# shenyunhang/JTSM

Measured on AMD Instinct MI355X. Metric: images/sec training, R50-FPN JTSM panoptic, 2x1024x1024, 1/2/4/8 GPU, higher is better.
Workload: dtype bf16x3; 1 GPU; BASELINE configs[2]: JTSM panoptic R50-FPN, 2 x 3x1024x1024 per GPU, 2000 proposals + 1024 superpixels per image; MIL + 4 OICR + 2 mask heads + sem-seg; fwd + bwd + gradient exchange + SGD; 100% of proposals jittered copies of 40 rectangles per image; global_batch=2, parallelism=dp1, foreground_rois_last_step=281

## Files before the change

include/jtsm_hip.h:

```cpp
#ifndef JTSM_HIP_H_
#define JTSM_HIP_H_

#include <stddef.h>
#include <stdint.h>

#ifdef __cplusplus
extern "C" {
#endif

#define JTSM_OK 0
#define JTSM_EINVAL (-1)
#define JTSM_ELAUNCH (-2)
#define JTSM_ENODEV (-3)

#define JTSM_NCHW 0
#define JTSM_NHWC 1

const char* jtsm_last_error(void);
const char* jtsm_version(void);
int jtsm_device_count(void);

void* jtsm_event_create(void);
int jtsm_event_record(void* event, void* stream);
int jtsm_event_elapsed_ms(void* start, void* stop, float* ms);
void jtsm_event_destroy(void* event);
void jtsm_conv_set_mid_event(void* event);
void jtsm_conv_set_splitk_fused(int mode);

int jtsm_roi_align_forward_f32(const float* input, const float* rois, float* output, int B,
                               int C, int H, int W, int M, float spatial_scale, int pooled_h,
                               int pooled_w, int sampling_ratio, int aligned, int layout,
                               void* stream);
int jtsm_roi_align_backward_f32(const float* grad, const float* rois, float* grad_input, int B,
                                int C, int H, int W, int M, float spatial_scale, int pooled_h,
                                int pooled_w, int sampling_ratio, int aligned, int layout,
                                void* stream);
int jtsm_roi_align_forward_f64(const double* input, const double* rois, double* output, int B,
                               int C, int H, int W, int M, double spatial_scale, int pooled_h,
                               int pooled_w, int sampling_ratio, int aligned, int layout,
                               void* stream);
int jtsm_roi_align_backward_f64(const double* grad, const double* rois, double* grad_input,
                                int B, int C, int H, int W, int M, double spatial_scale,
                                int pooled_h, int pooled_w, int sampling_ratio, int aligned,
                                int layout, void* stream);

int jtsm_roi_align_rotated_forward_f32(const float* input, const float* rois, float* output,
                                       int B, int C, int H, int W, int M, float spatial_scale,
                                       int pooled_h, int pooled_w, int sampling_ratio,
                                       int layout, void* stream);
int jtsm_roi_align_rotated_backward_f32(const float* grad, const float* rois, float* grad_input,
                                        int B, int C, int H, int W, int M, float spatial_scale,
                                        int pooled_h, int pooled_w, int sampling_ratio,
                                        int layout, void* stream);
int jtsm_roi_align_rotated_forward_f64(const double* input, const double* rois, double* output,
                                       int B, int C, int H, int W, int M, double spatial_scale,
                                       int pooled_h, int pooled_w, int sampling_ratio,
                                       int layout, void* stream);
int jtsm_roi_align_rotated_backward_f64(const double* grad, const double* rois,
                                        double* grad_input, int B, int C, int H, int W, int M,
                                        double spatial_scale, int pooled_h, int pooled_w,
                                        int sampling_ratio, int layout, void* stream);

int jtsm_roi_sample_table_f32(const float* rois, int rotated, int M, int H, int W,
                              float spatial_scale, int pooled_h, int pooled_w,
                              int sampling_ratio, int aligned, int* grid, int* pos, float* w,
                              int cap, void* stream);

size_t jtsm_moi_pool_workspace_bytes(int B, int H, int W, int M, int L);
int jtsm_moi_pool_forward_f32(const float* input, const float* rois, const int32_t* oh_labels,
                              const int32_t* superpixels, float* output, int32_t* argmax,
                              void* workspace, int B, int C, int H, int W, int M, int L, int Hs,
                              int Ws, float spatial_scale, int pooled_h, int pooled_w,
                              int layout, void* stream);
int jtsm_moi_pool_backward_f32(const float* grad, const float* rois, const int32_t* argmax,
                               float* grad_input, int B, int C, int H, int W, int M,
                               int pooled_h, int pooled_w, int layout, void* stream);
int jtsm_roi_loop_pool_forward_f32(const float* input, const float* rois, float* output, int32_t* argmax,
                                   int B, int C, int H, int W, int R, float spatial_scale, int pooled_h,
                                   int pooled_w, int layout, void* stream);
size_t jtsm_roi_loop_pool_backward_workspace_bytes(int R);
int jtsm_roi_loop_pool_backward_f32(const float* grad, const float* rois, const int32_t* argmax,
                                    float* grad_input, void* workspace, int B, int C, int H, int W, int R,
                                    float spatial_scale, int pooled_h, int pooled_w, void* stream);
int jtsm_roi_pool_forward_f32(const float* input, const float* rois, float* output, int32_t* argmax,
                              int B, int C, int H, int W, int R, float spatial_scale, int pooled_h,
                              int pooled_w, int layout, void* stream);
size_t jtsm_roi_pool_backward_workspace_bytes(int R);
int jtsm_roi_pool_backward_f32(const float* grad, const float* rois, const int32_t* argmax,
                               float* grad_input, void* workspace, int B, int C, int H, int W, int R,
                               float spatial_scale, int pooled_h, int pooled_w, void* stream);
size_t jtsm_pool_f16_workspace_bytes(long in_elems, long roi_elems, long out_elems, size_t extra);
size_t jtsm_moi_pool_f16_workspace_bytes(int B, int C, int H, int W, int M, int L, int pooled_h, int pooled_w);
int jtsm_roi_align_forward_f16(const uint16_t* input, const uint16_t* rois, uint16_t* output, int B, int C, int H, int W,
                               int M, float spatial_scale, int pooled_h, int pooled_w, int sampling_ratio, int aligned,
                               int layout, void* workspace, size_t workspace_bytes, void* stream);
int jtsm_roi_align_backward_f16(const uint16_t* grad, const uint16_t* rois, uint16_t* grad_input, int B, int C, int H,
                                int W, int M, float spatial_scale, int pooled_h, int pooled_w, int sampling_ratio,
                                int aligned, int layout, void* workspace, size_t workspace_bytes, void* stream);
int jtsm_roi_align_rotated_forward_f16(const uint16_t* input, const uint16_t* rois, uint16_t* output, int B, int C,
                                       int H, int W, int M, float spatial_scale, int pooled_h, int pooled_w,
                                       int sampling_ratio, int layout, void* workspace, size_t workspace_bytes,
                                       void* stream);
int jtsm_roi_align_rotated_backward_f16(const uint16_t* grad, const uint16_t* rois, uint16_t* grad_input, int B, int C,
                                        int H, int W, int M, float spatial_scale, int pooled_h, int pooled_w,
                                        int sampling_ratio, int layout, void* workspace, size_t workspace_bytes,
                                        void* stream);
int jtsm_moi_pool_forward_f16(const uint16_t* input, const uint16_t* rois, const int32_t* oh_labels,
                              const int32_t* superpixels, uint16_t* output, int32_t* argmax, void* workspace,
                              size_t workspace_bytes, int B, int C, int H, int W, int M, int L, int Hs, int Ws,
                              float spatial_scale, int pooled_h, int pooled_w, int layout, void* stream);
int jtsm_moi_pool_backward_f16(const uint16_t* grad, const uint16_t* rois, const int32_t* argmax, uint16_t* grad_input,
                               void* workspace, size_t workspace_bytes, int B, int C, int H, int W, int M, int pooled_h,
                               int pooled_w, int layout, void* stream);

size_t jtsm_moi_pool_levels_workspace_bytes(int B, const int* H, const int* W, int nlevels, int M, int L);
int jtsm_moi_pool_forward_levels_f32(const float* const* inputs, const int* H, const int* W,
                                     const float* scales, int nlevels, const float* rois,
                                     const int32_t* roi_level, const int32_t* oh_labels,
                                     const int32_t* superpixels, float* output, int32_t* argmax,
                                     void* workspace, int B, int C, int M, int L, int Hs, int Ws,
                                     int pooled_h, int pooled_w, void* stream);
size_t jtsm_moi_pool_backward_levels_workspace_bytes(const int* H, const int* W, int nlevels, int B, int M);
int jtsm_moi_pool_backward_levels_f32(const float* grad, const float* rois, const int32_t* roi_level,
                                      const int32_t* argmax, float* const* grad_inputs, const int* H,
                                      const int* W, const float* scales, int nlevels, int B, int C, int M,
                                      int pooled_h, int pooled_w, int accumulate, void* workspace,
                                      size_t workspace_bytes, void* stream);

int jtsm_moi_mask_f32(const float* rois, const int32_t* oh_labels, const int32_t* superpixels,
                      int32_t* mois, void* workspace, int B, int H, int W, int M, int L, int Hs,
                      int Ws, float spatial_scale, void* stream);


typedef struct jtsm_conv_shape {
  int batch, in_h, in_w, in_c;
  int out_c;
  int kernel_h, kernel_w;
  int stride, pad, dilation;
} jtsm_conv_shape;

int jtsm_conv_out_size(const jtsm_conv_shape* s, int* out_h, int* out_w);
size_t jtsm_conv_workspace_bytes(const jtsm_conv_shape* s, int backward_data);
int jtsm_conv_plan(const jtsm_conv_shape* s, int role, int has_kscale, int* kernel, int* tile_m,
                   int* tile_n, int* splits);

int jtsm_conv2d_forward_f32(const float* x, const float* w, float* y, const jtsm_conv_shape* s,
                            const float* scale, const float* bias, const float* residual,
                            int relu, void* workspace, size_t workspace_bytes, void* stream);
int jtsm_conv2d_backward_data_f32(const float* dy, const float* w, float* dx,
                                  const jtsm_conv_shape* s, const float* kscale,
                                  const float* accumulate, const float* relu_mask, void* workspace,
                                  size_t workspace_bytes, void* stream);
int jtsm_conv2d_backward_weight_f32(const float* dy, const float* x, float* dw,
                                    const jtsm_conv_shape* s, const float* row_scale, int zero_dw,
                                    void* stream);

int jtsm_split_bf16_f32(const float* src, uint16_t* hi, uint16_t* lo, long n, void* stream);
int jtsm_split_bf16_paired_f32(const float* src, uint16_t* planes, long rows, int k, void* stream);
int jtsm_split_bf16_transposed_f32(const float* w, const float* row_scale, uint16_t* hi, uint16_t* lo,
                                   int out_c, int taps, int in_c, void* stream);
int jtsm_split_bf16_multi_f32(const void* table, int entries, long blocks, int transposed, void* stream);
int jtsm_conv_bf16x3_eligible(const jtsm_conv_shape* s, int role);
int jtsm_conv_bf16x3_plan(const jtsm_conv_shape* s, int role, int* wm, int* wn, int* tm, int* tn, int* nbuf,
                          int* splits);
int jtsm_conv2d_forward_bf16x3(const uint16_t* x_hi, const uint16_t* x_lo, const uint16_t* w_hi,
                               const uint16_t* w_lo, float* y, uint16_t* y_hi, uint16_t* y_lo,
                               const jtsm_conv_shape* s, const float* scale, const float* bias,
                               const float* residual, int relu, void* workspace, size_t workspace_bytes,
                               void* stream);
int jtsm_conv2d_backward_data_bf16x3(const uint16_t* dy_hi, const uint16_t* dy_lo, const uint16_t* wt_hi,
                                     const uint16_t* wt_lo, float* dx, uint16_t* dx_hi, uint16_t* dx_lo,
                                     const jtsm_conv_shape* s, const float* accumulate,
                                     const float* relu_mask, void* workspace, size_t workspace_bytes,
                                     void* stream);
size_t jtsm_conv_bf16x3_wgrad_workspace_bytes(const jtsm_conv_shape* s);
int jtsm_conv2d_backward_weight_bf16x3(const uint16_t* dy_hi, const uint16_t* dy_lo, const uint16_t* x_hi,
                                       const uint16_t* x_lo, float* dw, const jtsm_conv_shape* s,
                                       const float* row_scale, int zero_dw, void* workspace,
                                       size_t workspace_bytes, void* stream);

int jtsm_split_f16_f32(const float* src, uint16_t* h, long n, int shift, void* stream);
int jtsm_split_f16_transposed_f32(const float* w, const float* row_scale, uint16_t* h, int out_c, int taps, int in_c,
                                  void* stream);
int jtsm_conv2d_forward_f16(const uint16_t* x_h, const uint16_t* w_h, float* y, uint16_t* y_h,
                            const jtsm_conv_shape* s, const float* scale, const float* bias,
                            const float* residual, int relu, void* workspace, size_t workspace_bytes,
                            void* stream);
int jtsm_conv2d_backward_data_f16(const uint16_t* dy_h, const uint16_t* wt_h, float* dx, uint16_t* dx_h,
                                  const jtsm_conv_shape* s, const float* accumulate, const float* relu_mask,
                                  int grad_shift, void* workspace, size_t workspace_bytes, void* stream);
int jtsm_conv2d_backward_weight_f16(const uint16_t* dy_h, const uint16_t* x_h, float* dw, const jtsm_conv_shape* s,
                                    const float* row_scale, int zero_dw, int grad_shift, void* workspace,
                                    size_t workspace_bytes, void* stream);
int jtsm_conv_transpose2x2_forward_bf16x3(const uint16_t* x_hi, const uint16_t* x_lo, const uint16_t* wt_hi,
                                          const uint16_t* wt_lo, float* y, uint16_t* y_hi, uint16_t* y_lo, int batch,
                                          int h, int w, int in_c, int out_c, const float* bias, int relu, void* stream);
int jtsm_conv_transpose2x2_forward_f16(const uint16_t* x_h, const uint16_t* wt_h, float* y, uint16_t* y_h, int batch,
                                       int h, int w, int in_c, int out_c, const float* bias, int relu, void* stream);
size_t jtsm_conv_transpose2x2_workspace_bytes(int batch, int h, int w, int in_c, int out_c);
int jtsm_conv_transpose2x2_backward_data_bf16x3(const uint16_t* g_hi, const uint16_t* g_lo, const uint16_t* w_hi,
                                                const uint16_t* w_lo, float* dx, uint16_t* dx_hi, uint16_t* dx_lo,
                                                int batch, int h, int w, int in_c, int out_c, const float* relu_mask,
                                                const uint16_t* gate_plane, void* workspace, size_t workspace_bytes,
                                                void* stream);
int jtsm_conv_transpose2x2_backward_data_f16(const uint16_t* g_h, const uint16_t* w_h, float* dx, uint16_t* dx_h,
                                             int batch, int h, int w, int in_c, int out_c, const float* relu_mask,
                                             const uint16_t* gate_plane, int grad_shift, void* workspace,
                                             size_t workspace_bytes, void* stream);
int jtsm_conv2d_backward_data_ex_bf16x3(const uint16_t* dy_hi, const uint16_t* dy_lo, const uint16_t* wt_hi,
                                        const uint16_t* wt_lo, float* dx, uint16_t* dx_hi, uint16_t* dx_lo,
                                        const jtsm_conv_shape* s, const float* row_scale, const float* accumulate,
                                        const float* relu_mask, const uint16_t* gate_plane, void* workspace,
                                        size_t workspace_bytes, void* stream);
int jtsm_conv2d_backward_data_ex_f16(const uint16_t* dy_h, const uint16_t* wt_h, float* dx, uint16_t* dx_h,
                                     const jtsm_conv_shape* s, const float* row_scale, const float* accumulate,
                                     const float* relu_mask, const uint16_t* gate_plane, int grad_shift, void* workspace,
                                     size_t workspace_bytes, void* stream);

int jtsm_conv2d_forward_res16_f16(const uint16_t* x_h, const uint16_t* w_h, float* y, uint16_t* y_h,
                                  const jtsm_conv_shape* s, const float* scale, const float* bias,
                                  const uint16_t* residual_h, int relu, void* workspace, size_t workspace_bytes,
                                  void* stream);
int jtsm_conv2d_backward_data_acc16_f16(const uint16_t* dy_h, const uint16_t* wt_h, float* dx, uint16_t* dx_h,
                                        const jtsm_conv_shape* s, const float* row_scale, const uint16_t* accumulate_h,
                                        const uint16_t* gate_plane, int grad_shift, void* workspace,
                                        size_t workspace_bytes, void* stream);

int jtsm_conv_bf16x3_colsum_rows(const jtsm_conv_shape* s, int role);
int jtsm_conv2d_backward_data_colsum_bf16x3(const uint16_t* dy_hi, const uint16_t* dy_lo, const uint16_t* wt_hi,
                                            const uint16_t* wt_lo, float* dx, uint16_t* dx_hi, uint16_t* dx_lo,
                                            const jtsm_conv_shape* s, const float* row_scale, const float* accumulate,
                                            const float* relu_mask, const uint16_t* gate_plane, float* colsum,
                                            void* workspace, size_t workspace_bytes, void* stream);
int jtsm_conv2d_backward_data_colsum_f16(const uint16_t* dy_h, const uint16_t* wt_h, float* dx, uint16_t* dx_h,
                                         const jtsm_conv_shape* s, const float* row_scale, const float* accumulate,
                                         const float* relu_mask, const uint16_t* gate_plane, int grad_shift, float* colsum,
                                         void* workspace, size_t workspace_bytes, void* stream);
int jtsm_conv_transpose2x2_backward_data_colsum_bf16x3(const uint16_t* g_hi, const uint16_t* g_lo, const uint16_t* w_hi,
                                                       const uint16_t* w_lo, float* dx, uint16_t* dx_hi, uint16_t* dx_lo,
                                                       int batch, int h, int w, int in_c, int out_c,
                                                       const float* relu_mask, const uint16_t* gate_plane, float* colsum,
                                                       void* workspace, size_t workspace_bytes, void* stream);
int jtsm_conv_transpose2x2_backward_data_colsum_f16(const uint16_t* g_h, const uint16_t* w_h, float* dx, uint16_t* dx_h,
                                                    int batch, int h, int w, int in_c, int out_c, const float* relu_mask,
                                                    const uint16_t* gate_plane, int grad_shift, float* colsum,
                                                    void* workspace, size_t workspace_bytes, void* stream);
int jtsm_relu_backward_split_scaled_f32(const float* dy, const float* y, float scale, float* g, uint16_t* g_hi,
                                        uint16_t* g_lo, long n, int shift, void* stream);
int jtsm_split_rowscale_f32(const float* src, const float* row_scale, long rows, int cols, uint16_t* hi, uint16_t* lo,
                            int shift, void* stream);
int jtsm_dropout_split_f32(const float* x, float* y, uint16_t* y_hi, uint16_t* y_lo, long n, float p,
                           unsigned long long seed, void* stream);
int jtsm_channel_sum_planes(const uint16_t* hi, const uint16_t* lo, float* out, long rows, int C, int shift,
                            void* workspace, size_t workspace_bytes, void* stream);
int jtsm_channel_sum_planes_multi(const uint16_t* const* hi, const uint16_t* const* lo, float* const* outs,
                                  const long* rows, int count, int C, int shift, void* workspace,
                                  size_t workspace_bytes, void* stream);
size_t jtsm_conv_bf16x3_wgrad_bias_workspace_bytes(const jtsm_conv_shape* s);
int jtsm_conv2d_backward_weight_bias_bf16x3(const uint16_t* dy_hi, const uint16_t* dy_lo, const uint16_t* x_hi,
                                            const uint16_t* x_lo, float* dw, float* db, const jtsm_conv_shape* s,
                                            const float* row_scale, int zero_dw, void* workspace,
                                            size_t workspace_bytes, void* stream);
int jtsm_conv2d_backward_weight_bias_f16(const uint16_t* dy_h, const uint16_t* x_h, float* dw, float* db,
                                         const jtsm_conv_shape* s, const float* row_scale, int zero_dw, int grad_shift,
                                         void* workspace, size_t workspace_bytes, void* stream);
size_t jtsm_conv_bf16x3_wgrad_group_workspace_bytes(const jtsm_conv_shape* s, int n);
int jtsm_conv_bf16x3_wgrad_group_plan(const jtsm_conv_shape* s, int n, int* tile, int* splits);
int jtsm_conv2d_backward_weight_group_bf16x3(int n, const uint16_t* const* dy_hi, const uint16_t* const* dy_lo,
                                             const uint16_t* const* x_hi, const uint16_t* const* x_lo,
                                             float* const* dw, const float* const* row_scale,
                                             const jtsm_conv_shape* s, void* workspace, size_t workspace_bytes,
                                             void* stream);
int jtsm_conv2d_backward_weight_group_f16(int n, const uint16_t* const* dy_h, const uint16_t* const* x_h,
                                          float* const* dw, const float* const* row_scale, const jtsm_conv_shape* s,
                                          int grad_shift, void* workspace, size_t workspace_bytes, void* stream);
int jtsm_relu_backward_split_f16(const float* dy, const float* y, float* g, uint16_t* g_h, long n, int shift,
                                 void* stream);

int jtsm_relu_backward_split_f32(const float* dy, const float* y, float* g, uint16_t* g_hi, uint16_t* g_lo,
                                 long n, void* stream);
int jtsm_relu_backward_f32(const float* dy, const float* y, float* g, long n, void* stream);
int jtsm_channel_sum_f32(const float* g, float* out, long rows, int C, void* stream);
int jtsm_colsum_fold_f32(const float* const* parts, const int* rows, int n, int width, float* out, void* stream);
size_t jtsm_channel_sum_workspace_bytes(long rows, int C);
int jtsm_channel_sum_ws_f32(const float* g, float* out, long rows, int C, void* workspace, size_t workspace_bytes,
                            void* stream);
int jtsm_sgd_momentum_multi_f32(const void* table, int entries, long blocks, int first_step, void* stream);


int jtsm_maxpool3x3s2_forward_f32(const float* x, float* y, int N, int H, int W, int C, void* stream);
int jtsm_maxpool3x3s2_backward_f32(const float* x, const float* gy, float* gx, int N, int H, int W,
                                   int C, void* stream);
int jtsm_maxpool2x2_forward_f32(const float* x, float* y, int N, int H, int W, int C, int stride, void* stream);
int jtsm_maxpool2x2_backward_f32(const float* x, const float* gy, float* gx, int N, int H, int W, int C,
                                 int stride, void* stream);
int jtsm_upsample2_add_f32(const float* top, const float* lateral, float* out, uint16_t* out_hi, uint16_t* out_lo,
                           int N, int H, int W, int C, void* stream);
int jtsm_sum_tensors_f32(const float* const* inputs, int n, long numel, float* out, uint16_t* out_hi, uint16_t* out_lo,
                         void* stream);
int jtsm_sum2x2_f32(const float* g, float* out, int N, int Ht, int Wt, int C, void* stream);
int jtsm_subsample2_f32(const float* src, float* dst, int N, int H, int W, int C, int scatter,
                        void* stream);


size_t jtsm_mil_workspace_bytes(int nbags, int max_bag_rows, int nc);
int jtsm_mil_forward_f32(const float* cls_logits, const float* det_logits, int ld, int nc,
                         const int32_t* bag_offsets, int nbags, int max_bag_rows,
                         const float* labels, int mean_loss, float* scores, float* img_probs,
                         float* loss, void* workspace, void* stream);
int jtsm_mil_backward_f32(const float* cls_logits, const float* det_logits, int ld, int nc,
                          const int32_t* bag_offsets, int nbags, int max_bag_rows,
                          const float* upstream, float* d_cls, float* d_det, int ld_grad,
                          const void* workspace, void* stream);

size_t jtsm_oicr_workspace_bytes(void);
int jtsm_oicr_forward_f32(const float* cls_logits, int ld_cls, int num_cls, const float* box_deltas,
                          int ld_box, const int32_t* labels, const float* weights,
                          const float* proposals, const float* gt_boxes, int R, float* losses,
                          void* workspace, void* stream);
int jtsm_oicr_backward_f32(const float* cls_logits, int ld_cls, int num_cls, const float* box_deltas,
                           int ld_box, const int32_t* labels, const float* weights,
                           const float* proposals, const float* gt_boxes, int R, const float* losses,
                           const float* up_cls, const float* up_box, float* d_cls, int ld_dcls,
                           float* d_box, int ld_dbox, void* stream);

int jtsm_oicr_smooth_forward_f32(const float* cls_logits, int ld_cls, int num_cls, const float* box_deltas,
                                 int ld_box, const int32_t* labels, const float* weights,
                                 const float* proposals, const float* gt_boxes, int R, float beta,
                                 float* losses, void* workspace, void* stream);
int jtsm_oicr_smooth_backward_f32(const float* cls_logits, int ld_cls, int num_cls, const float* box_deltas,
                                  int ld_box, const int32_t* labels, const float* weights,
                                  const float* proposals, const float* gt_boxes, int R, float beta,
                                  const float* losses, const float* up_cls, const float* up_box, float* d_cls,
                                  int ld_dcls, float* d_box, int ld_dbox, void* stream);


size_t jtsm_pcl_cluster_workspace_bytes(int nimg, int max_rows);
int jtsm_pcl_cluster_f32(const float* boxes, const int32_t* offsets, int nimg, int max_rows, int total_rows,
                         const float* prev_probs, int ld_prev, int prev_col0, const float* labels,
                         int num_classes, const float* probs, int ld_probs, int32_t* row_label,
                         int32_t* row_assign, float* row_weight, int32_t* pc_int, float* pc_flt,
                         int32_t* pc_num, void* workspace, void* stream);
int jtsm_pcl_softmax_f32(const float* logits, int ld, int num_cls, int R, float* probs, void* stream);
size_t jtsm_pcl_loss_workspace_bytes(int nimg);
int jtsm_pcl_loss_forward_f32(const float* probs, int ld_probs, const int32_t* offsets, int nimg,
                              int num_classes, const int32_t* row_label, const float* row_weight,
                              const int32_t* pc_int, const float* pc_flt, const int32_t* pc_num,
                              float* loss, void* workspace, void* stream);
int jtsm_pcl_loss_backward_f32(const float* logits, int ld, int num_classes, const int32_t* offsets,
                               int nimg, int total_rows, const int32_t* row_label,
                               const int32_t* row_assign, const float* row_weight, const int32_t* pc_int,
                               const float* pc_flt, const float* upstream, float* d_logits, int ld_grad,
                               void* stream);


int jtsm_rect_mask_targets_f32(const float* rois, const float* rects, uint8_t* out, int N, int side, int H, int W,
                               float erode, void* stream);
int jtsm_sp_mask_targets_f32(const float* rois, const int32_t* oh_row, const int32_t* img_of, const int32_t* oh_labels,
                             int L, const int32_t* superpixels, uint8_t* out, int N, int side, int H, int W,
                             void* stream);
int jtsm_paste_crop_targets_f32(const float* probs, const float* rois, uint8_t* out, int N, int M, int side, int H,
                                int W, float threshold, void* stream);
int jtsm_near_targets_f32(const float* proposals, const int32_t* bag_offsets, int B, int R, const int32_t* labels,
                          int bg_label, const float* pgt_box, const int32_t* counts, int Gmax, int top_k,
                          int32_t* near_rows, int32_t* matched_near, void* stream);

int jtsm_pooler_rois_levels_f32(const float* const* boxes, const int* counts, int B, int min_level, int max_level,
                                float canonical_box_size, float canonical_level, float* rois, int32_t* level,
                                void* stream);
int jtsm_roi_scale_f32(const int32_t* argmax, int bins, int C, const float* const* objectness, const int* counts, int B,
                       float* out, void* stream);
size_t jtsm_image_labels_workspace_bytes(int B);
int jtsm_image_labels(const int64_t* const* gt_classes, const int* counts, int B, int num_classes, const void* sem_seg,
                      int sem_elem_bytes, long pixels, int num_stuff, int stuff_offset, float* oh_things,
                      int32_t* things_cls, int32_t* things_cnt, float* oh_stuff, int32_t* stuff_cls, int32_t* stuff_cnt,
                      void* workspace, void* stream);

int jtsm_fg_compact(const int32_t* labels, int bg_label, const int32_t* bag_offsets, int B, int R, const float* boxes,
                    const int32_t* matched, int32_t* fg_rows, float* fg_boxes, int64_t* fg_classes, int32_t* fg_img,
                    int32_t* fg_matched, float* fg_rois, int64_t* counts, void* stream);

size_t jtsm_mask_bce_workspace_bytes(void);
int jtsm_mask_bce_forward_f32(const float* logits, int ld, int num_classes, const int64_t* gt_classes,
                              const uint8_t* target, int N, int side, float* out, void* workspace,
                              void* stream);
int jtsm_mask_bce_backward_f32(const float* logits, int ld, int num_classes, const int64_t* gt_classes,
                               const uint8_t* target, int N, int side, const float* upstream,
                               float* dlogits, void* stream);


int jtsm_roi_align_forward_level_f32(const float* input, const float* rois,
                                     const int32_t* roi_level, int level, float* output, int B,
                                     int C, int H, int W, int M, float spatial_scale, int pooled_h,
                                     int pooled_w, int sampling_ratio, int aligned, void* stream);
int jtsm_roi_align_backward_level_f32(const float* grad, const float* rois,
                                      const int32_t* roi_level, int level, float* grad_input, int B,
                                      int C, int H, int W, int M, float spatial_scale, int pooled_h,
                                      int pooled_w, int sampling_ratio, int aligned, void* stream);
int jtsm_roi_align_rotated_forward_level_f32(const float* input, const float* rois, const int32_t* roi_level,
                                             int level, float* output, int B, int C, int H, int W, int M,
                                             float spatial_scale, int pooled_h, int pooled_w, int sampling_ratio,
                                             void* stream);
int jtsm_roi_align_rotated_backward_level_f32(const float* grad, const float* rois, const int32_t* roi_level,
                                              int level, float* grad_input, int B, int C, int H, int W, int M,
                                              float spatial_scale, int pooled_h, int pooled_w, int sampling_ratio,
                                              int accumulate, void* stream);
size_t jtsm_roi_align_backward_levels_workspace_bytes(const int* H, const int* W, int nlevels, int B, int C, int M);
int jtsm_roi_align_backward_levels_f32(const float* grad, const float* rois, const int32_t* roi_level,
                                       float* const* grad_inputs, const int* H, const int* W, const float* scales,
                                       int nlevels, int B, int C, int M, int pooled_h, int pooled_w, int sampling_ratio,
                                       int aligned, int accumulate, void* workspace, size_t workspace_bytes,
                                       void* stream);
int jtsm_moi_pool_forward_level_f32(const float* input, const float* rois, const int32_t* roi_level,
                                    int level, const int32_t* oh_labels, const int32_t* superpixels,
                                    float* output, int32_t* argmax, void* workspace, int B, int C,
                                    int H, int W, int M, int L, int Hs, int Ws, float spatial_scale,
                                    int pooled_h, int pooled_w, void* stream);
int jtsm_moi_pool_backward_level_f32(const float* grad, const float* rois, const int32_t* roi_level,
                                     int level, const int32_t* argmax, float* grad_input, int B, int C,
                                     int H, int W, int M, int pooled_h, int pooled_w, void* stream);


size_t jtsm_group_norm_workspace_bytes(int N, long HW, int C);
int jtsm_group_norm_forward_f32(const float* x, const float* gamma, const float* beta, float* y,
                                float* mean, float* rstd, void* workspace, int N, long HW, int C, int G,
                                float eps, int relu, void* stream);
int jtsm_group_norm_backward_f32(const float* x, const float* dy, const float* gamma, const float* beta,
                                 const float* mean, const float* rstd, float* dx, uint16_t* dx_hi,
                                 uint16_t* dx_lo, float* dgamma, float* dbeta, void* workspace, int N, long HW,
                                 int C, int G, int relu, void* stream);
int jtsm_upsample_bilinear2x_forward_f32(const float* x, float* y, uint16_t* y_hi, uint16_t* y_lo, int N, int H,
                                         int W, int C, void* stream);
int jtsm_upsample_bilinear2x_backward_f32(const float* gy, float* gx, int N, int H, int W, int C,
                                          void* stream);


size_t jtsm_semseg_ce_workspace_bytes(int N, int Hs, int Ws, int S);
int jtsm_semseg_ce_forward_f32(const float* logits, int ld, int C, const int64_t* target, float* out,
                               void* workspace, int N, int Hs, int Ws, int S, long ignore_index,
                               void* stream);
int jtsm_semseg_ce_backward_f32(const float* logits, int ld, int C, const int64_t* target,
                                const float* fwd_out, const float* upstream, float* dlogits,
                                const void* workspace, int N, int Hs, int Ws, int S, long ignore_index,
                                void* stream);


int jtsm_row_lse_f32(const float* logits, int ld, int ncls, int R, float* lse, void* stream);
int jtsm_mine_top1_f32(const float* scores, int ld, const float* lse, const float* proposals,
                       const float* deltas, int ld_deltas, const int32_t* bag_offsets,
                       const int32_t* classes, const int32_t* counts, int B, int Gmax,
                       const float* img_probs, int nprob, int32_t* out_idx, float* out_box,
                       float* out_score, float* out_weight, void* stream);
size_t jtsm_paint_sem_seg_workspace_bytes(int B);
int jtsm_paint_sem_seg(const float* boxes, const int32_t* classes, const float* scores, const int32_t* counts,
                       int B, int G, int class_base, int H, int W, float erode, int64_t* out, void* workspace,
                       void* stream);
int jtsm_paint_sem_seg_evidence(const int32_t* target_idx, const int32_t* bag_offsets, const int32_t* oh_labels, int L,
                                const int32_t* superpixels, const int32_t* classes, const float* scores,
                                const int32_t* counts, int B, int G, int class_base, int H, int W, int64_t* out,
                                void* workspace, void* stream);
int jtsm_match_label_f32(const float* proposals, const int32_t* bag_offsets, int B, int R,
                         const float* pgt_box, const int32_t* classes, const int32_t* counts,
                         const float* pgt_weight, const float* pgt_score, int Gmax, float iou_thresh,
                         int bg_label, int32_t* labels, int32_t* matched, float* gt_boxes,
                         float* gt_weights, float* gt_scores, void* stream);

size_t jtsm_mine_top_p_workspace_bytes(int B, int G, int t_max);
int jtsm_mine_top_p_f32(const float* scores, int ld, const float* lse, const float* proposals,
                        const float* deltas, int ld_deltas, int decode_zero_deltas,
                        const int32_t* bag_offsets, const int32_t* classes, const int32_t* counts,
                        const int32_t* top_t, int B, int G, int t_max, float iou_thresh, float* out_boxes,
                        int32_t* out_classes, float* out_scores, float* out_weights, int32_t* out_rows,
// ... 79 lines not shown
```

jtsm_amd/_lib.py:

```python
import ctypes as C
import os
import re

import torch

_HERE = os.path.dirname(os.path.abspath(__file__))
LIB_PATH = os.environ.get("JTSM_HIP_LIB") or os.path.join(_HERE, "lib", "libjtsm_hip.so")
HEADER = os.path.join(_HERE, "..", "include", "jtsm_hip.h")
_lib = None

NCHW, NHWC = 0, 1

_SCALARS = {"int": C.c_int, "int32_t": C.c_int, "unsigned": C.c_uint, "long": C.c_long, "size_t": C.c_size_t,
            "int64_t": C.c_int64, "unsigned long long": C.c_ulonglong, "float": C.c_float, "double": C.c_double}
_RETURNS = dict(_SCALARS, **{"void": None, "void*": C.c_void_p, "const char*": C.c_char_p})


def declarations(path=HEADER):
    txt = open(path).read()
    txt = re.sub(r"/\*.*?\*/|//[^\n]*", " ", txt, flags=re.S)
    txt = re.sub(r"^\s*#.*$", " ", txt, flags=re.M)
    out = {}
    for m in re.finditer(r"([\w\s*]+?)\b(jtsm_\w+)\s*\(([^()]*)\)\s*;", txt):
        ret, name, params = re.sub(r"\s*\*\s*", "*", " ".join(m.group(1).split())), m.group(2), m.group(3)
        decl = " ".join(m.group(0).split())
        if ret not in _RETURNS:
            raise ValueError("jtsm_amd: no ctypes mapping for the return type of `%s`" % decl)
        argtypes = []
        for p in params.split(","):
            words = re.sub(r"\bconst\b", " ", p).split()
            if "*" in p:
                argtypes.append(C.c_void_p)
            elif words != ["void"]:
                t = _SCALARS.get(" ".join(words[:-1]))
                if t is None:
                    raise ValueError("jtsm_amd: no ctypes mapping for `%s` in `%s`" % (p.strip(), decl))
                argtypes.append(t)
        out[name] = (_RETURNS[ret], argtypes)
    return out


def lib():
    global _lib
    if _lib is None:
        if not os.path.isfile(LIB_PATH):
            raise RuntimeError(
                "jtsm_amd: %s not found — build it with `python -m jtsm_amd.build` "
                "(there is no fallback path)" % LIB_PATH)
        raw = C.CDLL(LIB_PATH)
        for name, (restype, argtypes) in declarations().items():
            fn = getattr(raw, name, None)
            if fn is None:
                raise RuntimeError("jtsm_amd: %s lacks %s, which include/jtsm_hip.h declares" % (LIB_PATH, name))
            fn.restype, fn.argtypes = restype, argtypes
        _lib = raw
    if TIMING is not None:
        return _TimedLib(_lib)
    return _lib


TIMING = None
_pending_bytes = None
_UNTIMED = ("jtsm_event_", "jtsm_last_error", "jtsm_version", "jtsm_device_count", "jtsm_conv_set_mid_event",
            "jtsm_conv_set_splitk_fused", "jtsm_conv_plan", "jtsm_conv_bf16x3_plan", "jtsm_conv_bf16x3_eligible", "jtsm_conv_out_size",
            "jtsm_conv2d_", "jtsm_conv_transpose2x2_")


def note_bytes(nbytes):
    global _pending_bytes
    if TIMING is not None:
        _pending_bytes = float(nbytes)


class EventSpan(object):
    __slots__ = ("a", "b")

    def __init__(self, raw):
        self.a, self.b = raw.jtsm_event_create(), raw.jtsm_event_create()

    def ms(self):
        out = C.c_float()
        return out.value if lib().jtsm_event_elapsed_ms(self.a, self.b, C.byref(out)) == 0 else 0.0

    def __del__(self):
        try:
            for e in (self.a, self.b):
                lib().jtsm_event_destroy(e)
        except Exception:
            pass


class _TimedLib(object):
    def __init__(self, raw):
        self._raw = raw

    def __getattr__(self, name):
        fn = getattr(self._raw, name)
        if TIMING is None or name.endswith("_workspace_bytes") or name.startswith(_UNTIMED):
            return fn
        raw = self._raw

        def timed(*args):
            global _pending_bytes
            span = EventSpan(raw)
            st = stream()
            raw.jtsm_event_record(span.a, st)
            rc = fn(*args)
            raw.jtsm_event_record(span.b, st)
            TIMING.append((name, span, _pending_bytes))
            _pending_bytes = None
            return rc
        return timed


def check(rc, what=""):
    if rc != 0:
        msg = lib().jtsm_last_error().decode("utf-8", "replace")
        raise RuntimeError("jtsm_hip %s failed (%d): %s" % (what, rc, msg))


def ptr(t):
    return None if t is None else t.data_ptr()


_raw_stream = getattr(torch._C, "_cuda_getCurrentRawStream", None)
_device_index = None


def stream():
    global _device_index
    if _raw_stream is None:
        return torch.cuda.current_stream().cuda_stream
    if _device_index is None:
        _device_index = torch.cuda.current_device()
    return _raw_stream(_device_index)


def _check_device(t):
    if _device_index is not None and t.device.index is not None and t.device.index != _device_index:
        raise RuntimeError("jtsm_amd: this process launches on cuda:%d but got a tensor on %s (one process per GPU)"
                           % (_device_index, t.device))


def require_gpu(*tensors):
    for t in tensors:
        if t is not None and not t.is_cuda:
            raise RuntimeError(
                "jtsm_amd operators run only on the HIP device (got a %s tensor); "
                "there is no CPU path in the product" % t.device)
        if t is not None:
            _check_device(t)


def is_nhwc(t):
    return t.dim() == 4 and t.is_contiguous(memory_format=torch.channels_last) and not (
        t.is_contiguous() and t.shape[1] != 1 and t.shape[2] * t.shape[3] != 1)
```

jtsm_amd/modeling/backbone/resnet.py:

```python
import torch
import torch.nn.functional as F
from torch import nn

from ...layers.grad_fan import fan_out
from ...layers.batch_norm import FrozenBatchNorm2d, get_norm
from ...layers.blocks import CNNBlockBase
from ...layers.elementwise import max_pool_3x3_s2
from ...layers import fused_blocks
from ...layers.fused_blocks import bottleneck_fused
from ...layers.wrappers import Conv2d
from .backbone import Backbone
from .build import BACKBONE_REGISTRY

BLOCKS_PER_STAGE = {18: (2, 2, 2, 2), 34: (3, 4, 6, 3), 50: (3, 4, 6, 3), 101: (3, 4, 23, 3), 152: (3, 8, 36, 3)}
_STAGE_NUMBER = {"res2": 2, "res3": 3, "res4": 4, "res5": 5}


def _msra(conv):
    nn.init.kaiming_normal_(conv.weight, mode="fan_out", nonlinearity="relu")
    if conv.bias is not None:
        nn.init.constant_(conv.bias, 0)


def conv_norm(cin, cout, k, norm, *, stride=1, dilation=1, relu=False):
    conv = Conv2d(cin, cout, kernel_size=k, stride=stride, padding=(k // 2) * dilation, dilation=dilation, bias=False,
                  norm=get_norm(norm, cout), activation=F.relu if relu else None)
    _msra(conv)
    return conv


def _all_frozen(convs):
    return all(isinstance(c.norm, FrozenBatchNorm2d) and c.bias is None for c in convs)


class BasicBlock(CNNBlockBase):

    def __init__(self, in_channels, out_channels, *, stride=1, norm="BN"):
        super().__init__(in_channels, out_channels, stride)
        self.shortcut = None
        if in_channels != out_channels:
            self.shortcut = conv_norm(in_channels, out_channels, 1, norm, stride=stride)
        self.conv1 = conv_norm(in_channels, out_channels, 3, norm, stride=stride, relu=True)
        self.conv2 = conv_norm(out_channels, out_channels, 3, norm, relu=True)

    def forward(self, x):
        skip = x if self.shortcut is None else self.shortcut(x)
        return self.conv2(self.conv1(x), residual=skip)


class BottleneckBlock(CNNBlockBase):

    def __init__(self, in_channels, out_channels, *, bottleneck_channels, stride=1, num_groups=1, norm="BN",
                 stride_in_1x1=False, dilation=1):
        super().__init__(in_channels, out_channels, stride)
        if num_groups != 1:
            raise NotImplementedError("jtsm_amd BottleneckBlock: num_groups=1 only")
        s1, s3 = (stride, 1) if stride_in_1x1 else (1, stride)
        mid = bottleneck_channels
        self.shortcut = None
        if in_channels != out_channels:
            self.shortcut = conv_norm(in_channels, out_channels, 1, norm, stride=stride)
        self.conv1 = conv_norm(in_channels, mid, 1, norm, stride=s1, relu=True)
        self.conv2 = conv_norm(mid, mid, 3, norm, stride=s3, dilation=dilation, relu=True)
        self.conv3 = conv_norm(mid, out_channels, 1, norm, relu=True)

    def _members(self):
        return [c for c in (self.conv1, self.conv2, self.conv3, self.shortcut) if c is not None]

    def forward(self, x):
        if fused_blocks.ENABLED and x.is_cuda and x.dtype == torch.float32 and x.shape[1] % 8 == 0 and \
                _all_frozen(self._members()):
            sc = self.shortcut
            return bottleneck_fused(
                x, self.conv1.weight, self.conv1.norm.scale_bias(), self.conv2.weight, self.conv2.norm.scale_bias(),
                self.conv3.weight, self.conv3.norm.scale_bias(), sc.weight if sc is not None else None,
                sc.norm.scale_bias() if sc is not None else None, self.conv1.stride[0], self.conv2.stride[0],
                self.conv2.padding[0], self.conv2.dilation[0], sc.stride[0] if sc is not None else 1)
        skip = x if self.shortcut is None else self.shortcut(x)
        return self.conv3(self.conv2(self.conv1(x)), residual=skip)


class BasicStem(CNNBlockBase):

    def __init__(self, in_channels=3, out_channels=64, norm="BN"):
        super().__init__(in_channels, out_channels, 4)
        self.in_channels = in_channels
        self.conv1 = conv_norm(in_channels, out_channels, 7, norm, stride=2, relu=True)

    def forward(self, x):
        return max_pool_3x3_s2(self.conv1(x))


class ResNet(Backbone):

    def __init__(self, stem, stages, num_classes=None, out_features=None, pad_to_stride=False):
        super().__init__()
        if num_classes is not None:
            raise NotImplementedError("the classification head is outside the JTSM path")
        self.stem = stem
        channels, strides = {"stem": stem.out_channels}, {"stem": stem.stride}
        stride, order = stem.stride, []
        for number, blocks in enumerate(stages, start=2):
            blocks = list(blocks)
            if not blocks:
                raise ValueError("ResNet: stage res%d has no blocks" % number)
            name = "res%d" % number
            self.add_module(name, nn.Sequential(*blocks))
            for b in blocks:
                stride *= b.stride
            channels[name], strides[name] = blocks[-1].out_channels, stride
            order.append(name)
        self.stage_names = tuple(order)
        wanted = list(out_features) if out_features else [order[-1]]
        unknown = [f for f in wanted if f not in channels]
        if unknown:
            raise ValueError("ResNet: unknown out_features %s (have %s)" % (unknown, sorted(channels)))
        self._declare_outputs(wanted, {f: channels[f] for f in wanted}, {f: strides[f] for f in wanted})
        self._size_divisibility = stride if pad_to_stride else 0

    @property
    def size_divisibility(self):
        return self._size_divisibility

    @property
    def stages(self):
        return [getattr(self, n) for n in self.stage_names]

    def forward(self, x):
        if x.dim() != 4:
            raise ValueError("ResNet takes an input of shape (N, C, H, W), got %s" % (tuple(x.shape),))
        keep = set(self._out_features)
        out = {}
        x = self.stem(x)
        if "stem" in keep:
            out["stem"] = x
        for name in self.stage_names:
            x = self._run_stage(getattr(self, name), x)
            if name in keep:
                if name != self.stage_names[-1]:
                    out[name], x = fan_out(x, 2)
                else:
                    out[name] = x
        return out

    @staticmethod
    def _run_stage(stage, x):
        blocks = list(stage.children())
        rest = blocks[1:]
        if rest and all(isinstance(b, BottleneckBlock) and _all_frozen(b._members()) for b in blocks) and \
                fused_blocks.identity_chain_ok(x, rest):
            y = blocks[0](x)
            if fused_blocks.identity_chain_ok(y, rest):
                return fused_blocks.identity_chain_fused(y, rest)
            for b in rest:
                y = b(y)
            return y
        return stage(x)

    def freeze(self, freeze_at=0):
        if freeze_at >= 1:
            self.stem.freeze()
        for name in self.stage_names:
            if freeze_at >= _STAGE_NUMBER[name]:
                for block in getattr(self, name).children():
                    block.freeze()
        return self

    @staticmethod
    def make_stage(block_class, num_blocks, first_stride=None, *, in_channels, out_channels, **kwargs):
        if first_stride is not None:
            if "stride" in kwargs or "stride_per_block" in kwargs:
                raise ValueError("make_stage: give first_stride or stride(_per_block), not both")
            kwargs["stride_per_block"] = [first_stride] + [1] * (num_blocks - 1)
        suffix = "_per_block"
        varying = {k[:-len(suffix)]: v for k, v in kwargs.items() if k.endswith(suffix)}
        shared = {k: v for k, v in kwargs.items() if not k.endswith(suffix)}
        for k, v in varying.items():
            if len(v) != num_blocks:
                raise ValueError("make_stage: %s%s has %d entries for %d blocks" % (k, suffix, len(v), num_blocks))
        blocks, cin = [], in_channels
        for i in range(num_blocks):
            blocks.append(block_class(in_channels=cin, out_channels=out_channels, **shared,
                                      **{k: v[i] for k, v in varying.items()}))
            cin = out_channels
        return blocks


def resnet_cfg(cfg):
    r = cfg.MODEL.RESNETS
    if r.DEPTH not in BLOCKS_PER_STAGE:
        raise ValueError("MODEL.RESNETS.DEPTH must be one of %s, got %r" % (sorted(BLOCKS_PER_STAGE), r.DEPTH))
    if any(r.DEFORM_ON_PER_STAGE):
        raise NotImplementedError("deformable conv is outside the JTSM path (SURVEY 2.1)")
    assert r.RES5_DILATION in {1, 2}, "res5_dilation cannot be {}.".format(r.RES5_DILATION)
    if r.DEPTH in (18, 34):
        assert r.RES2_OUT_CHANNELS == 64, "Must set MODEL.RESNETS.RES2_OUT_CHANNELS = 64 for R18/R34"
        assert r.NUM_GROUPS == 1, "Must set MODEL.RESNETS.NUM_GROUPS = 1 for R18/R34"
    last = max(_STAGE_NUMBER[f] for f in r.OUT_FEATURES if f != "stem")
    return r, BLOCKS_PER_STAGE[r.DEPTH][:last - 1]


@BACKBONE_REGISTRY.register()
def build_resnet_backbone(cfg, input_shape):
    r, counts = resnet_cfg(cfg)
    basic = r.DEPTH in (18, 34)
    if basic:
        assert r.RES5_DILATION == 1, "Must set MODEL.RESNETS.RES5_DILATION = 1 for R18/R34"
    stem = BasicStem(in_channels=input_shape.channels, out_channels=r.STEM_OUT_CHANNELS, norm=r.NORM)
    cin, cout, mid = r.STEM_OUT_CHANNELS, r.RES2_OUT_CHANNELS, r.NUM_GROUPS * r.WIDTH_PER_GROUP
    stages = []
    for number, n in enumerate(counts, start=2):
        dilated = number == 5 and r.RES5_DILATION == 2
        first_stride = 1 if (number == 2 or dilated) else 2
        if basic:
            stage = ResNet.make_stage(BasicBlock, n, first_stride, in_channels=cin, out_channels=cout, norm=r.NORM)
        else:
            stage = ResNet.make_stage(BottleneckBlock, n, first_stride, in_channels=cin, out_channels=cout,
                                      norm=r.NORM, bottleneck_channels=mid, stride_in_1x1=r.STRIDE_IN_1X1,
                                      dilation=2 if dilated else 1, num_groups=r.NUM_GROUPS)
        stages.append(stage)
        cin, cout, mid = cout, cout * 2, mid * 2
    return ResNet(stem, stages, out_features=r.OUT_FEATURES).freeze(cfg.MODEL.BACKBONE.FREEZE_AT)
```

Before: 97.44 images/sec.

## Fuse ResNet stem conv7x7, frozen BN, ReLU and maxpool into one MFMA kernel

Adds a HIP kernel that computes the 7x7 stride-2 stem convolution with bf16x3 MFMA, applies frozen-BN scale/bias and ReLU, then does the 3x3 stride-2 max pool from LDS. It also writes the bf16 hi/lo planes directly. The goal is to avoid writing the full-resolution conv output to memory, along with separate split and pool launches. The path runs only when grad is not needed for the input or the stem weight, which holds for a frozen stem in training. Each workgroup recomputes the overlapping halo around its tile, and the path adds a new large kernel to maintain.

```diff
diff --git a/include/jtsm_hip.h b/include/jtsm_hip.h
--- a/include/jtsm_hip.h
+++ b/include/jtsm_hip.h
@@ -168,6 +168,8 @@
                                const jtsm_conv_shape* s, const float* scale, const float* bias,
                                const float* residual, int relu, void* workspace, size_t workspace_bytes,
                                void* stream);
+int jtsm_stem_forward_bf16x3(const float* x, const float* w, const float* scale, const float* bias, float* y,
+                             uint16_t* y_hi, uint16_t* y_lo, int N, int H, int W, int C, int out_c, void* stream);
 int jtsm_conv2d_backward_data_bf16x3(const uint16_t* dy_hi, const uint16_t* dy_lo, const uint16_t* wt_hi,
                                      const uint16_t* wt_lo, float* dx, uint16_t* dx_hi, uint16_t* dx_lo,
                                      const jtsm_conv_shape* s, const float* accumulate,
diff --git a/jtsm_amd/_lib.py b/jtsm_amd/_lib.py
--- a/jtsm_amd/_lib.py
+++ b/jtsm_amd/_lib.py
@@ -63,7 +63,7 @@
 _pending_bytes = None
 _UNTIMED = ("jtsm_event_", "jtsm_last_error", "jtsm_version", "jtsm_device_count", "jtsm_conv_set_mid_event",
             "jtsm_conv_set_splitk_fused", "jtsm_conv_plan", "jtsm_conv_bf16x3_plan", "jtsm_conv_bf16x3_eligible", "jtsm_conv_out_size",
-            "jtsm_conv2d_", "jtsm_conv_transpose2x2_")
+            "jtsm_conv2d_", "jtsm_conv_transpose2x2_", "jtsm_stem_forward_")
 
 
 def note_bytes(nbytes):
diff --git a/jtsm_amd/csrc/stem_x3.hip b/jtsm_amd/csrc/stem_x3.hip
--- /dev/null
+++ b/jtsm_amd/csrc/stem_x3.hip
@@ -0,0 +1,286 @@
+#include <cfloat>
+
+#include "common.h"
+
+namespace jtsm {
+namespace {
+
+typedef __bf16 bf16x8 __attribute__((ext_vector_type(8)));
+typedef __bf16 bf16x4 __attribute__((ext_vector_type(4)));
+typedef float f32x16 __attribute__((ext_vector_type(16)));
+
+constexpr int TP = 8;
+constexpr int TC = 2 * TP + 1;
+constexpr int PH = 2 * (TC - 1) + 7;
+constexpr int PW = 2 * (TC - 1) + 8;
+constexpr int NPIX = TC * TC;
+constexpr int NBLK = (NPIX + 31) / 32;
+constexpr int KK = 7 * 32;
+constexpr int COUT = 64;
+constexpr int NT = 512, NWAVE = 8;
+constexpr int QW = NWAVE / 2;
+constexpr int MAXB = (NBLK + QW - 1) / QW;
+static_assert(NBLK - QW * (MAXB - 1) == QW / 2, "wavefronts w and w + 4 share a SIMD: 3 + 2 blocks on each");
+constexpr int FETCH = (PH * PW + NT - 1) / NT;
+constexpr int W_PLANE = KK * COUT * 2;
+constexpr int P_PLANE = PH * PW * 8;
+constexpr int CONV_B = NPIX * COUT * 4;
+constexpr int LDSB = 2 * W_PLANE + 2 * P_PLANE + CONV_B;
+static_assert(LDSB <= 160 * 1024, "one workgroup must fit the CU's LDS");
+static_assert(P_PLANE % 16 == 0 && W_PLANE % 16 == 0, "16-byte aligned LDS regions");
+
+__device__ __forceinline__ void split1(float v, __bf16& h, __bf16& l) {
+  h = (__bf16)v;
+  l = (__bf16)(v - (float)h);
+}
+
+struct StemArgs {
+  const float* x;
+  const float* w;
+  const float* scale;
+  const float* bias;
+  float* y;
+  unsigned short* y_hi;
+  unsigned short* y_lo;
+  int N, H, W;
+  int Ho, Wo;
+  int Hp, Wp;
+  int tiles_y, tiles_x, tiles;
+};
+
+template <int C>
+__device__ __forceinline__ void patch_fetch(const StemArgs& a, int tile, int t, float (&v)[FETCH][4]) {
+  const int tx = tile % a.tiles_x, r = tile / a.tiles_x;
+  const int ty = r % a.tiles_y, n = r / a.tiles_y;
+  const int iy0 = 4 * TP * ty - 5, ix0 = 4 * TP * tx - 5;
+#pragma unroll
+  for (int i = 0; i < FETCH; ++i) {
+    const int q = t + NT * i;
+    const int iy = iy0 + q / PW, ix = ix0 + q % PW;
+    v[i][0] = v[i][1] = v[i][2] = v[i][3] = 0.f;
+    if (q < PH * PW && (unsigned)iy < (unsigned)a.H && (unsigned)ix < (unsigned)a.W) {
+      const float* s = a.x + (((size_t)n * a.H + iy) * a.W + ix) * C;
+      if (C == 4) {
+        const float4 f = *reinterpret_cast<const float4*>(s);
+        v[i][0] = f.x; v[i][1] = f.y; v[i][2] = f.z; v[i][3] = f.w;
+      } else {
+        v[i][0] = s[0]; v[i][1] = s[1]; v[i][2] = s[2];
+      }
+    }
+  }
+}
+
+__device__ __forceinline__ void patch_store(char* p_hi, char* p_lo, int t, const float (&v)[FETCH][4]) {
+#pragma unroll
+  for (int i = 0; i < FETCH; ++i) {
+    const int q = t + NT * i;
+    if (q >= PH * PW) continue;
+    bf16x4 h, l;
+#pragma unroll
+    for (int e = 0; e < 4; ++e) {
+      __bf16 hh, ll;
+      split1(v[i][e], hh, ll);
+      h[e] = hh; l[e] = ll;
+    }
+    *reinterpret_cast<bf16x4*>(p_hi + q * 8) = h;
+    *reinterpret_cast<bf16x4*>(p_lo + q * 8) = l;
+  }
+}
+
+template <int NB>
+__device__ __forceinline__ void mma_phase(const char* w_hi, const char* w_lo, const char* p_hi, const char* p_lo,
+                                          int wave, int lane, f32x16 (&acc)[MAXB]) {
+  const int r = lane & 31, h = lane >> 5, cb = wave & 1;
+  int aoff[NB];
+#pragma unroll
+  for (int i = 0; i < NB; ++i) {
+    int p = ((wave >> 1) + QW * i) * 32 + r;
+    p = p < NPIX ? p : NPIX - 1;
+    const int oy = p / TC, ox = p % TC;
+    aoff[i] = ((2 * oy) * PW + 2 * ox + 2 * h) * 8;
+  }
+#pragma unroll
+  for (int i = 0; i < NB; ++i)
+#pragma unroll
+    for (int e = 0; e < 16; ++e) acc[i][e] = 0.f;
+  const int boff = (h * COUT + cb * 32 + r) * 16;
+#pragma unroll
+  for (int s = 0; s < KK / 16; ++s) {
+    const int koff = ((s >> 1) * PW + 4 * (s & 1)) * 8;
+    const bf16x8 bh = *reinterpret_cast<const bf16x8*>(w_hi + boff + 2 * s * COUT * 16);
+    const bf16x8 bl = *reinterpret_cast<const bf16x8*>(w_lo + boff + 2 * s * COUT * 16);
+#pragma unroll
+    for (int i = 0; i < NB; ++i) {
+      const bf16x8 ah = *reinterpret_cast<const bf16x8*>(p_hi + aoff[i] + koff);
+      const bf16x8 al = *reinterpret_cast<const bf16x8*>(p_lo + aoff[i] + koff);
+      acc[i] = __builtin_amdgcn_mfma_f32_32x32x16_bf16(al, bh, acc[i], 0, 0, 0);
+      acc[i] = __builtin_amdgcn_mfma_f32_32x32x16_bf16(ah, bl, acc[i], 0, 0, 0);
+      acc[i] = __builtin_amdgcn_mfma_f32_32x32x16_bf16(ah, bh, acc[i], 0, 0, 0);
+    }
+  }
+}
+
+template <int NB>
+__device__ __forceinline__ void conv_store(float* conv, const f32x16 (&acc)[MAXB], int wave, int lane, int cy0, int cx0,
+                                           int Ho, int Wo, float sc, float bi) {
+  const int r = lane & 31, h = lane >> 5, cb = wave & 1;
+#pragma unroll
+  for (int i = 0; i < NB; ++i) {
+    int p0 = ((wave >> 1) + QW * i) * 32 + 4 * h;
+    asm volatile("" : "+v"(p0));
+    const int oy0 = p0 / TC, ox0 = p0 - oy0 * TC;
+    float* const dst = conv + p0 * COUT + cb * 32 + r;
+#pragma unroll
+    for (int e = 0; e < 16; ++e) {
+      const int d = (e & 3) + 8 * (e >> 2);
+      int ox = ox0 + d, oy = oy0;
+      if (ox >= TC) { ox -= TC; ++oy; }
+      if (ox >= TC) { ox -= TC; ++oy; }
+      if (p0 + d >= NPIX) continue;
+      const bool in = (unsigned)(cy0 + oy) < (unsigned)Ho && (unsigned)(cx0 + ox) < (unsigned)Wo;
+      float v = acc[i][e];
+      v = v * sc + bi;
+      v = fmaxf(v, 0.f);
+      dst[d * COUT] = in ? v : -FLT_MAX;
+    }
+  }
+}
+
+__device__ __forceinline__ float4 f4max(const float4& a, const float4& b) {
+  return make_float4(fmaxf(a.x, b.x), fmaxf(a.y, b.y), fmaxf(a.z, b.z), fmaxf(a.w, b.w));
+}
+
+template <int C>
+__global__ __launch_bounds__(NT) void stem_x3_kernel(const StemArgs a) {
+  __shared__ __attribute__((aligned(16))) char lds[LDSB];
+  char* const w_hi = lds;
+  char* const w_lo = lds + W_PLANE;
+  char* const p_hi = lds + 2 * W_PLANE;
+  char* const p_lo = p_hi + P_PLANE;
+  float* const conv = reinterpret_cast<float*>(p_lo + P_PLANE);
+  const int t = threadIdx.x, lane = t & 63, wave = t >> 6;
+
+  int tile = blockIdx.x;
+  if (tile >= a.tiles) return;
+  float pre[FETCH][4];
+  patch_fetch<C>(a, tile, t, pre);
+
+  constexpr int WBATCH = 14;
+  static_assert(COUT * KK % (NT * WBATCH) == 0, "");
+#pragma unroll 1
+  for (int base = t; base < COUT * KK; base += NT * WBATCH) {
+    float v[WBATCH];
+#pragma unroll
+    for (int j = 0; j < WBATCH; ++j) {
+      const int idx = base + NT * j;
+      const int n = idx / KK, k = idx % KK;
+      const int ky = k >> 5, kx = (k & 31) >> 2, c = k & 3;
+      v[j] = (kx < 7 && c < C) ? a.w[((n * 7 + ky) * 7 + kx) * C + c] : 0.f;
+    }
+#pragma unroll
+    for (int j = 0; j < WBATCH; ++j) {
+      const int idx = base + NT * j;
+      const int n = idx / KK, k = idx % KK;
+      __bf16 hh, ll;
+      split1(v[j], hh, ll);
+      const int o = (((k >> 3) * COUT + n) * 8 + (k & 7)) * 2;
+      *reinterpret_cast<__bf16*>(w_hi + o) = hh;
+      *reinterpret_cast<__bf16*>(w_lo + o) = ll;
+    }
+  }
+  const float sc = a.scale[(wave & 1) * 32 + (lane & 31)], bi = a.bias[(wave & 1) * 32 + (lane & 31)];
+
+  for (; tile < a.tiles; tile += gridDim.x) {
+    const int tx = tile % a.tiles_x, rr = tile / a.tiles_x;
+    const int ty = rr % a.tiles_y, n = rr / a.tiles_y;
+    patch_store(p_hi, p_lo, t, pre);
+    __syncthreads();
+    const int next = tile + gridDim.x;
+    if (next < a.tiles) patch_fetch<C>(a, next, t, pre);
+
+    f32x16 acc[MAXB];
+    const int cy0 = 2 * TP * ty - 1, cx0 = 2 * TP * tx - 1;
+    if ((wave >> 1) + QW * (MAXB - 1) < NBLK) {
+      mma_phase<MAXB>(w_hi, w_lo, p_hi, p_lo, wave, lane, acc);
+      conv_store<MAXB>(conv, acc, wave, lane, cy0, cx0, a.Ho, a.Wo, sc, bi);
+    } else {
+      mma_phase<MAXB - 1>(w_hi, w_lo, p_hi, p_lo, wave, lane, acc);
+      conv_store<MAXB - 1>(conv, acc, wave, lane, cy0, cx0, a.Ho, a.Wo, sc, bi);
+    }
+    __syncthreads();
+
+#pragma unroll
+    for (int it = 0; it < TP * TP * (COUT / 4) / NT; ++it) {
+      const int item = t + NT * it;
+      const int c4 = item & 15, pp = item >> 4;
+      const int py = pp / TP, px = pp % TP;
+      const int gy = TP * ty + py, gx = TP * tx + px;
+      if (gy >= a.Hp || gx >= a.Wp) continue;
+      float4 m = make_float4(-FLT_MAX, -FLT_MAX, -FLT_MAX, -FLT_MAX);
+#pragma unroll
+      for (int dy = 0; dy < 3; ++dy)
+#pragma unroll
+        for (int dx = 0; dx < 3; ++dx)
+          m = f4max(m, *reinterpret_cast<const float4*>(conv + ((2 * py + dy) * TC + 2 * px + dx) * COUT + c4 * 4));
+      const size_t o = (((size_t)n * a.Hp + gy) * a.Wp + gx) * COUT + c4 * 4;
+      *reinterpret_cast<float4*>(a.y + o) = m;
+      const float v[4] = {m.x, m.y, m.z, m.w};
+      bf16x4 hv, lv;
+#pragma unroll
+      for (int e = 0; e < 4; ++e) {
+        __bf16 hh, ll;
+        split1(v[e], hh, ll);
+        hv[e] = hh; lv[e] = ll;
+      }
+      *reinterpret_cast<bf16x4*>(a.y_hi + o) = hv;
+      *reinterpret_cast<bf16x4*>(a.y_lo + o) = lv;
+    }
+  }
+}
+
+int cu_count() {
+  static int n = 0;
+  if (n == 0) {
+    int dev = 0, v = 0;
+    if (hipGetDevice(&dev) == hipSuccess &&
+        hipDeviceGetAttribute(&v, hipDeviceAttributeMultiprocessorCount, dev) == hipSuccess && v > 0)
+      n = v;
+    else
+      n = 256;
+  }
+  return n;
+}
+
+}
+}
+
+using namespace jtsm;
+
+extern "C" int jtsm_stem_forward_bf16x3(const float* x, const float* w, const float* scale, const float* bias, float* y,
+                                        uint16_t* y_hi, uint16_t* y_lo, int N, int H, int W, int C, int out_c,
+                                        void* stream) {
+  JTSM_REQUIRE(out_c == COUT, "stem: 64 output channels only (got %d)", out_c);
+  JTSM_REQUIRE(C == 3 || C == 4, "stem: 3 or 4 input channels (got %d)", C);
+  JTSM_REQUIRE(N >= 0 && H >= 7 && W >= 7, "stem: needs H, W >= 7 (got %d x %d x %d)", N, H, W);
+  if (N == 0) return JTSM_OK;
+  JTSM_REQUIRE(x && w && scale && bias && y && y_hi && y_lo, "stem: null pointer");
+  JTSM_REQUIRE(((uintptr_t)y | (uintptr_t)y_hi | (uintptr_t)y_lo) % 16 == 0 && (C != 4 || (uintptr_t)x % 16 == 0),
+               "stem: y and its planes (and a 4-channel x) must be 16-byte aligned");
+  StemArgs a;
+  a.x = x; a.w = w; a.scale = scale; a.bias = bias;
+  a.y = y; a.y_hi = y_hi; a.y_lo = y_lo;
+  a.N = N; a.H = H; a.W = W;
+  a.Ho = (H + 6 - 7) / 2 + 1; a.Wo = (W + 6 - 7) / 2 + 1;
+  a.Hp = (a.Ho + 2 - 3) / 2 + 1; a.Wp = (a.Wo + 2 - 3) / 2 + 1;
+  a.tiles_y = ceil_div(a.Hp, TP); a.tiles_x = ceil_div(a.Wp, TP);
+  const long tiles = (long)N * a.tiles_y * a.tiles_x;
+  JTSM_REQUIRE(tiles < (1L << 30), "stem: too many tiles");
+  a.tiles = (int)tiles;
+  const int grid = a.tiles < cu_count() ? a.tiles : cu_count();
+  if (C == 4)
+    hipLaunchKernelGGL(stem_x3_kernel<4>, dim3(grid), dim3(NT), 0, as_stream(stream), a);
+  else
+    hipLaunchKernelGGL(stem_x3_kernel<3>, dim3(grid), dim3(NT), 0, as_stream(stream), a);
+  JTSM_CHECK_LAUNCH("stem_x3");
+  return JTSM_OK;
+}
diff --git a/jtsm_amd/layers/stem.py b/jtsm_amd/layers/stem.py
--- /dev/null
+++ b/jtsm_amd/layers/stem.py
@@ -0,0 +1,54 @@
+import os
+
+import torch
+
+from .. import _lib as L
+from . import conv
+from .batch_norm import FrozenBatchNorm2d
+
+CL = torch.channels_last
+FUSED = os.environ.get("JTSM_STEM_FUSED", "1") != "0"
+
+
+def stem_fused_ok(conv1, x):
+    from .wrappers import _is_relu
+    if not (FUSED and conv.MATH == "bf16x3" and x.is_cuda and x.dtype == torch.float32 and x.dim() == 4):
+        return False
+    if torch.is_grad_enabled() and (x.requires_grad or conv1.weight.requires_grad):
+        return False
+    return (conv1.kernel_size == (7, 7) and conv1.stride == (2, 2) and conv1.padding == (3, 3)
+            and conv1.dilation == (1, 1) and conv1.bias is None and conv1.out_channels == 64
+            and isinstance(conv1.norm, FrozenBatchNorm2d) and _is_relu(conv1.activation)
+            and x.shape[1] == conv1.in_channels and x.shape[1] in (3, 4) and x.shape[2] >= 7 and x.shape[3] >= 7
+            and conv1.weight.dtype == torch.float32)
+
+
+def stem_forward_fused(conv1, x):
+    L.require_gpu(x, conv1.weight)
+    x = x.detach().contiguous(memory_format=CL)
+    w = conv1.weight.detach().contiguous(memory_format=CL)
+    scale, bias = conv1.norm.scale_bias()
+    scale, bias = scale.detach().contiguous(), bias.detach().contiguous()
+    n, c, h, wd = x.shape
+    o = w.shape[0]
+    ho, wo = (h - 1) // 2 + 1, (wd - 1) // 2 + 1
+    hp, wp = (ho - 1) // 2 + 1, (wo - 1) // 2 + 1
+    y = torch.empty((n, o, hp, wp), dtype=x.dtype, device=x.device, memory_format=CL)
+    buf = conv._planes_buf(y.numel(), y.device)
+    hi, lo = conv._hl(buf)
+    lib, st = L.lib(), L.stream()
+    log = conv.LAUNCH_LOG
+    if log is not None:
+        span = conv.LaunchSpan()
+        lib.jtsm_event_record(span.a, st)
+    L.check(lib.jtsm_stem_forward_bf16x3(L.ptr(x), L.ptr(w), L.ptr(scale), L.ptr(bias), L.ptr(y), hi, lo,
+                                         n, h, wd, c, o, st), "stem_forward_bf16x3")
+    if log is not None:
+        lib.jtsm_event_record(span.mid, st)
+        lib.jtsm_event_record(span.b, st)
+        variant = conv._Variant("stem_x3_kernel<%d>" % c)
+        variant.segment = conv.SEGMENT
+        nbytes = 4.0 * (x.numel() + w.numel()) + 8.0 * y.numel()
+        log.append((variant, 2.0 * n * ho * wo * o * c * 49, span, (n, h, wd, c, o, 7, 2, nbytes), 0.0))
+    conv.planes_put(y, buf)
+    return y
diff --git a/jtsm_amd/modeling/backbone/resnet.py b/jtsm_amd/modeling/backbone/resnet.py
--- a/jtsm_amd/modeling/backbone/resnet.py
+++ b/jtsm_amd/modeling/backbone/resnet.py
@@ -8,6 +8,7 @@
 from ...layers.elementwise import max_pool_3x3_s2
 from ...layers import fused_blocks
 from ...layers.fused_blocks import bottleneck_fused
+from ...layers.stem import stem_forward_fused, stem_fused_ok
 from ...layers.wrappers import Conv2d
 from .backbone import Backbone
 from .build import BACKBONE_REGISTRY
@@ -88,6 +89,8 @@
         self.conv1 = conv_norm(in_channels, out_channels, 7, norm, stride=2, relu=True)
 
     def forward(self, x):
+        if stem_fused_ok(self.conv1, x):
+            return stem_forward_fused(self.conv1, x)
         return max_pool_3x3_s2(self.conv1(x))
 
 
```

Result: no change. 98.30 images/sec, median of 6 (+0.9%).
